# choyingw/SynergyNet

Hardware: AMD Instinct MI355X
Metric: faces/sec (120x120, 68-lmk + 53215-vert) (higher is better)
Workload: dtype f32 (fp16x2 split operands, fp32 accumulate)

## Files before the change

synergynet_amd/csrc/fused_block_lb.hip:

```cpp
#include "syn_internal.h"

#include <cstdio>
#include <cstdlib>

namespace syn {

typedef float f32x4 __attribute__((ext_vector_type(4)));
typedef float f32x2 __attribute__((ext_vector_type(2)));
typedef unsigned u32x4 __attribute__((ext_vector_type(4)));
typedef unsigned u32x2 __attribute__((ext_vector_type(2)));
typedef _Float16 f16x8 __attribute__((ext_vector_type(8)));
typedef _Float16 f16x2 __attribute__((ext_vector_type(2)));

namespace {
__device__ __forceinline__ void split2h(float x0, float x1, unsigned &a, unsigned &b) {
    a = __builtin_bit_cast(unsigned, __builtin_amdgcn_cvt_pkrtz(x0, x1));
    float r0, r1;
    asm("v_fma_mix_f32 %0, %1, -1.0, %2 op_sel_hi:[1,0,0]" : "=v"(r0) : "v"(a), "v"(x0));
    asm("v_fma_mix_f32 %0, %1, -1.0, %2 op_sel:[1,0,0] op_sel_hi:[1,0,0]" : "=v"(r1) : "v"(a), "v"(x1));
    b = __builtin_bit_cast(unsigned, __builtin_amdgcn_cvt_pkrtz(r0, r1));
}
__device__ __forceinline__ void split2v(float x0, float x1, u32x4 (&pc)[2], int d) {
    unsigned a, b;
    split2h(x0, x1, a, b);
    pc[0][d] = a; pc[1][d] = b;
}
__device__ __forceinline__ f32x4 mfmal(u32x4 a, u32x4 b, f32x4 c) {
    return __builtin_amdgcn_mfma_f32_16x16x32_f16(__builtin_bit_cast(f16x8, a), __builtin_bit_cast(f16x8, b), c, 0, 0, 0);
}
__device__ __forceinline__ void mac3x4(const u32x4 (&a0)[2], const u32x4 (&b0)[2], f32x4 &c0, const u32x4 (&a1)[2], const u32x4 (&b1)[2], f32x4 &c1,
                                       const u32x4 (&a2)[2], const u32x4 (&b2)[2], f32x4 &c2, const u32x4 (&a3)[2], const u32x4 (&b3)[2], f32x4 &c3) {
    constexpr int PA[3] = {1, 0, 0}, PB[3] = {0, 1, 0};
#pragma unroll
    for (int j = 0; j < 3; ++j) {
        c0 = mfmal(a0[PA[j]], b0[PB[j]], c0);
        c1 = mfmal(a1[PA[j]], b1[PB[j]], c1);
        c2 = mfmal(a2[PA[j]], b2[PB[j]], c2);
        c3 = mfmal(a3[PA[j]], b3[PB[j]], c3);
    }
}
__device__ __forceinline__ u32x4 bload4(__amdgpu_buffer_rsrc_t rs, unsigned voff, int soff) {
    return __builtin_amdgcn_raw_buffer_load_b128(rs, voff, soff, 0);
}
__device__ __forceinline__ f32x4 bload4f(__amdgpu_buffer_rsrc_t rs, unsigned voff, int soff) {
    return __builtin_bit_cast(f32x4, __builtin_amdgcn_raw_buffer_load_b128(rs, voff, soff, 0));
}
template <int CTRL>
__device__ __forceinline__ float dpp1(float x) {
    return __builtin_bit_cast(float, __builtin_amdgcn_mov_dpp(__builtin_bit_cast(int, x), CTRL, 0xf, 0xf, true));
}
template <int CTRL>
__device__ __forceinline__ f32x2 dpp2(f32x2 v) {
    f32x2 r;
    r[0] = dpp1<CTRL>(v[0]);
    r[1] = dpp1<CTRL>(v[1]);
    return r;
}
__device__ __forceinline__ float relu01(float d, float m) { return __builtin_amdgcn_fmed3f(d * m, 0.0f, 1.0f); }
__device__ __forceinline__ f32x2 pk_fma_clamp01(f32x2 a, f32x2 b, f32x2 c) {
    f32x2 r;
    asm("v_pk_fma_f32 %0, %1, %2, %3 clamp" : "=v"(r) : "v"(a), "v"(b), "v"(c));
    return r;
}
constexpr int kRowShr1 = 0x111, kRowShl1 = 0x101, kRowShr8 = 0x118, kRowShl8 = 0x108;
constexpr int kRowShr4 = 0x114, kRowShr5 = 0x115;
}

template <int CIN_, int HID_, int COUT_, bool RES_, int EPF_, int PPF_, int FPW_ = 2, bool S2_ = false, int NS_ = 2>
struct LbCfg {
    static constexpr int CIN = CIN_, HID = HID_, COUT = COUT_, FPW = FPW_;
    static constexpr int PPF = PPF_;
    static constexpr bool TLATE = false;
    static constexpr int EPF = EPF_;
    static constexpr bool RES = RES_;
    static constexpr bool S2 = S2_;
    static constexpr int NB = S2 ? 1 : 4;
    static constexpr int PIXO = NB * 16;
    static constexpr int KE = CIN / 32;
    static constexpr int NG = HID / 32;
    static constexpr int MT = COUT / 16;
    static constexpr int NS = NS_;
    static constexpr int NW = FPW * NS, NT = NW * 64;
    static constexpr int XF_DW = KE * 4 * 2 * 256;
    static constexpr int NSX = NS == 8 ? 4 : NS;
    static constexpr int KT = (MT + NSX - 1) / NSX;
    static constexpr int RED_DW = (NS == 2 ? 1 : NSX) * MT * NB * 256;
    static constexpr int TB_DW = 12 * 32;
    static constexpr int FACE_DW = XF_DW > RED_DW ? XF_DW : RED_DW;
    static constexpr int LDS_DW = FPW * FACE_DW + NW * TB_DW;
    static_assert(CIN % 32 == 0 && HID % 64 == 0 && COUT % 32 == 0, "k32 steps, two streams, two halves of the output tiles");
    static_assert(NS == 2 || (NS == 8 && FPW == 1 && (HID / 32) >= NS), "eight streams: the one-face-per-workgroup schedule of small batches (the four-stream form of round 4 is retired)");
    static_assert(EPF == 1 || EPF == KE, "expand prefetch depth");
    static_assert(!RES || (CIN == COUT && !S2), "residual only on same-width stride-1 blocks");
    static_assert((FPW == 4 || NS >= 4 ? 1 : 2) * LDS_DW * 4 <= 160 * 1024, "one 8-wave or two 4-wave workgroups per CU");
};

#define SYNL_FENCE() do { asm volatile("" ::: "memory"); __builtin_amdgcn_sched_barrier(0); } while (0)

#define SYNL_LAP(i) do { if (PROF) { tn = __builtin_amdgcn_s_memtime(); pt_[i] += tn - tk; tk = tn; } } while (0)

struct LbStageArgs {
    const float *X;
    const unsigned *Weh;
    const float *Tlb;
    const unsigned *Wlb;
    const float *p_shift;
    float *Y;
    float *part = nullptr;
    int gsl = 0;
};

template <class C, class CN, bool FIRST, bool PROF, int FACE_DW, bool STORE = true, bool PARTIAL = false, int RED_OFF = 0>
__device__ __forceinline__ void lb_stage(unsigned *smem, const LbStageArgs &sa, int B, unsigned long long (&pt_)[5], unsigned long long &tk) {
    unsigned long long tn = 0;
    const float *__restrict__ X = sa.X;
    const unsigned *__restrict__ Weh = sa.Weh, *__restrict__ Wlb = sa.Wlb;
    const float *__restrict__ Tlb = sa.Tlb, *__restrict__ p_shift = sa.p_shift;
    float *__restrict__ Y = sa.Y;
    constexpr int KE = C::KE, MT = C::MT, CIN = C::CIN, COUT = C::COUT, NB = C::NB;
    const int tid = threadIdx.x, lane = tid & 63;
    const int wave = __builtin_amdgcn_readfirstlane(tid >> 6);
    const int fl = wave / C::NS, st = wave % C::NS;
    const int f = blockIdx.x * C::FPW + fl;
    const bool real = f < B;
    const int fc = real ? f : B - 1;
    const int n = lane & 15, g = lane >> 4;
    const unsigned l4 = lane * 4, g4 = g * 4;
    unsigned *Xf = smem + fl * FACE_DW;
    constexpr int BPW = 4 / C::NS;
    auto pix_in = [&](int b, int nn) __attribute__((always_inline)) {
        return C::S2 ? 16 * (nn >> 2) + 8 * (b >> 1) + 2 * (nn & 3) + (b & 1) : 32 * (nn >> 3) + (nn & 7) + 8 * b;
    };

    if constexpr (FIRST && C::NS == 8) {
        constexpr int NIT = (KE * 4 + 7) / 8;
        f32x4 xv[NIT][2];
#pragma unroll
        for (int i = 0; i < NIT; ++i) {
            const int it = st + 8 * i, itc = it < KE * 4 ? it : 0;
            const float *src = X + ((size_t)fc * 64 + pix_in(itc & 3, n)) * CIN + 32 * (itc >> 2) + 8 * g;
            xv[i][0] = *(const f32x4 *)src;
            xv[i][1] = *(const f32x4 *)(src + 4);
        }
#pragma unroll
        for (int i = 0; i < NIT; ++i) {
            const int it = st + 8 * i;
            f32x4 a = xv[i][0], b = xv[i][1];
            if (!real) { a = (f32x4){0.f, 0.f, 0.f, 0.f}; b = a; }
            a *= 16.0f; b *= 16.0f;
            u32x4 pc[2];
            split2v(a[0], a[1], pc, 0);
            split2v(a[2], a[3], pc, 1);
            split2v(b[0], b[1], pc, 2);
            split2v(b[2], b[3], pc, 3);
            if (it < KE * 4) {
#pragma unroll
                for (int p = 0; p < 2; ++p) *(u32x4 *)&Xf[(it * 2 + p) * 256 + lane * 4] = pc[p];
            }
        }
    } else if (FIRST) {
        f32x4 xv[KE][BPW][2];
#pragma unroll
        for (int kc = 0; kc < KE; ++kc)
#pragma unroll
            for (int rr = 0; rr < BPW; ++rr) {
                const float *src = X + ((size_t)fc * 64 + pix_in(BPW * st + rr, n)) * CIN + 32 * kc + 8 * g;
                xv[kc][rr][0] = *(const f32x4 *)src;
                xv[kc][rr][1] = *(const f32x4 *)(src + 4);
            }
#pragma unroll
        for (int kc = 0; kc < KE; ++kc)
#pragma unroll
            for (int rr = 0; rr < BPW; ++rr) {
                f32x4 a = xv[kc][rr][0], b = xv[kc][rr][1];
                if (!real) { a = (f32x4){0.f, 0.f, 0.f, 0.f}; b = a; }
                a *= 16.0f; b *= 16.0f;
                u32x4 pc[2];
                split2v(a[0], a[1], pc, 0);
                split2v(a[2], a[3], pc, 1);
                split2v(b[0], b[1], pc, 2);
                split2v(b[2], b[3], pc, 3);
#pragma unroll
                for (int p = 0; p < 2; ++p) *(u32x4 *)&Xf[((kc * 4 + BPW * st + rr) * 2 + p) * 256 + lane * 4] = pc[p];
            }
    }
    const float mL = (C::S2 ? (n & 3) : (n & 7)) != 0 ? 1.f : 0.f, mR = (C::S2 || (n & 7) != 7) ? 1.f : 0.f;
    f32x4 acc[MT][NB];
#pragma unroll
    for (int mt = 0; mt < MT; ++mt)
#pragma unroll
        for (int r = 0; r < NB; ++r) acc[mt][r] = (f32x4){0.f, 0.f, 0.f, 0.f};

    float *Tb = reinterpret_cast<float *>(smem + C::FPW * FACE_DW + wave * C::TB_DW);
    const __amdgpu_buffer_rsrc_t rs_e = __builtin_amdgcn_make_buffer_rsrc(const_cast<unsigned *>(Weh), 0, 0x7fffffff, 0x00027000);
    const __amdgpu_buffer_rsrc_t rs_p = __builtin_amdgcn_make_buffer_rsrc(const_cast<unsigned *>(Wlb), 0, 0x7fffffff, 0x00027000);
    const __amdgpu_buffer_rsrc_t rs_t = __builtin_amdgcn_make_buffer_rsrc(const_cast<float *>(Tlb), 0, 0x7fffffff, 0x00027000);
    const unsigned l16 = lane * 16;
    f32x4 tv[2];
    auto fetch_t = [&](int G) __attribute__((always_inline)) {
        tv[0] = bload4f(rs_t, l16, G * (C::TB_DW * 4));
        tv[1] = bload4f(rs_t, l16 & 511, G * (C::TB_DW * 4) + 1024);
    };
    auto park_t = [&]() __attribute__((always_inline)) {
        *(f32x4 *)&Tb[l4] = tv[0];
        *(f32x4 *)&Tb[256 + (l4 & 127)] = tv[1];
    };
    const float c6e = Tlb[11 * 32], inv_p = Tlb[11 * 32 + 1];
    u32x4 Ae[C::EPF == 1 ? 2 : KE][2][2];
    auto fetch_e = [&](int G, int kc) __attribute__((always_inline)) {
#pragma unroll
        for (int t = 0; t < 2; ++t)
#pragma unroll
            for (int p = 0; p < 2; ++p)
                Ae[kc % (C::EPF == 1 ? 2 : KE)][t][p] = bload4(rs_e, l16, G * (2 * KE * 2048) + ((t * KE + kc) * 2 + p) * 1024);
    };
    const int gb = PARTIAL ? (int)blockIdx.y * sa.gsl : 0, gend = PARTIAL ? gb + sa.gsl : C::NG;
    fetch_t(gb + st);
#pragma unroll
    for (int kc = 0; kc < C::EPF; ++kc) fetch_e(gb + st, kc);
    park_t();
    __syncthreads();
    SYNL_LAP(0);

    for (int G = gb + st; G < gend; G += C::NS) {
        f32x4 D[2][4];
#pragma unroll
        for (int t = 0; t < 2; ++t) {
            const f32x4 es = *(const f32x4 *)&Tb[10 * 32 + 16 * t + g4];
#pragma unroll
            for (int r = 0; r < 4; ++r) D[t][r] = es;
        }
#pragma unroll
        for (int kc = 0; kc < KE; ++kc) {
            if (kc + C::EPF < KE) fetch_e(G, kc + C::EPF);
            constexpr int SL = C::EPF == 1 ? 2 : KE;
#pragma unroll
            for (int r = 0; r < 4; r += 2) {
                u32x4 Bx[2][2];
#pragma unroll
                for (int rr = 0; rr < 2; ++rr)
#pragma unroll
                    for (int p = 0; p < 2; ++p) Bx[rr][p] = *(const u32x4 *)&Xf[((kc * 4 + r + rr) * 2 + p) * 256 + lane * 4];
                mac3x4(Ae[kc % SL][0], Bx[0], D[0][r], Ae[kc % SL][1], Bx[0], D[1][r], Ae[kc % SL][0], Bx[1], D[0][r + 1], Ae[kc % SL][1], Bx[1], D[1][r + 1]);
                SYNL_FENCE();
            }
        }
        if (C::EPF == KE && G + C::NS < gend) {
#pragma unroll
            for (int kc = 0; kc < C::EPF; ++kc) fetch_e(G + C::NS, kc);
        }
        SYNL_FENCE();
        SYNL_LAP(1);
        constexpr int RING = C::S2 ? 4 : C::PPF + 1;
        u32x4 Ap[RING][2];
        auto fetch_p = [&](int mt) __attribute__((always_inline)) {
#pragma unroll
            for (int p = 0; p < 2; ++p) Ap[mt % RING][p] = bload4(rs_p, l16, G * (MT * 2048) + (mt * 2 + p) * 1024);
        };
        u32x4 Bd[NB][2];
#pragma unroll
        for (int th = 0; th < 4; ++th) {
            const int t = th >> 1, hf = th & 1;
            if (th == 3) fetch_p(0);
            const int c0 = 16 * t + 2 * hf;
            f32x2 w[9];
#pragma unroll
            for (int k = 0; k < 9; ++k) w[k] = *(const f32x2 *)&Tb[k * 32 + c0 + g4];
            const f32x2 dsh = *(const f32x2 *)&Tb[9 * 32 + c0 + g4];
            if (C::S2) {
#pragma unroll
                for (int dy = 0; dy < 3; ++dy) { w[3 * dy] *= mL; w[3 * dy + 2] *= mR; }
            }
            f32x2 E[4], O[NB];
#pragma unroll
            for (int r = 0; r < 4; ++r) {
                E[r][0] = relu01(D[t][r][2 * hf], c6e);
                E[r][1] = relu01(D[t][r][2 * hf + 1], c6e);
            }
#pragma unroll
            for (int r = 0; r < NB; ++r) O[r] = dsh;
            if constexpr (C::S2) {
                O[0] += dpp2<kRowShr5>(E[3]) * w[0];
                O[0] += dpp2<kRowShr4>(E[2]) * w[1];
                O[0] += dpp2<kRowShr4>(E[3]) * w[2];
                asm volatile("" : "+v"(O[0]));
                O[0] += dpp2<kRowShr1>(E[1]) * w[3];
                O[0] += E[0] * w[4];
                O[0] += E[1] * w[5];
                asm volatile("" : "+v"(O[0]));
                O[0] += dpp2<kRowShr1>(E[3]) * w[6];
                O[0] += E[2] * w[7];
                O[0] = pk_fma_clamp01(E[3], w[8], O[0]);
            } else {
                const f32x2 mL2 = {mL, mL}, mR2 = {mR, mR};
                f32x2 rowT = E[3], rowB = E[0];
                asm volatile("" : "+v"(rowT), "+v"(rowB));
                rowT = dpp2<kRowShr8>(rowT);
                rowB = dpp2<kRowShl8>(rowB);
#pragma unroll
                for (int r = 0; r < 4; ++r) {
                    const f32x2 &i0 = r == 0 ? rowT : E[r - 1], &i1 = E[r], &i2 = r == 3 ? rowB : E[r + 1];
                    f32x2 A = i0 * w[0], Cc = i0 * w[2], Bc = O[r] + i0 * w[1];
                    A += i1 * w[3]; Bc += i1 * w[4]; Cc += i1 * w[5];
                    A += i2 * w[6]; Bc += i2 * w[7]; Cc += i2 * w[8];
                    Bc += dpp2<kRowShr1>(A) * mL2;
                    O[r] = pk_fma_clamp01(dpp2<kRowShl1>(Cc), mR2, Bc);
                    asm volatile("" : "+v"(O[r]));
                }
            }
#pragma unroll
            for (int r = 0; r < NB; ++r) {
                split2v(O[r][0], O[r][1], Bd[r], th);
                if (hf) {
#pragma unroll
                    for (int p = 0; p < 2; ++p) asm volatile("" : "+v"(Bd[r][p]));
                }
            }
            SYNL_FENCE();
        }
        SYNL_LAP(2);
        const bool more = G + C::NS < gend;
#pragma unroll
        for (int i = 1; i < C::PPF; ++i)
            if (i < MT) fetch_p(i);
        if (more) {
            if (!C::TLATE) fetch_t(G + C::NS);
            if (C::EPF != KE) {
#pragma unroll
                for (int kc = 0; kc < C::EPF; ++kc) fetch_e(G + C::NS, kc);
            }
        }
        if constexpr (C::S2) {
            static_assert(!C::S2 || (C::PPF == 2 && MT % 2 == 0), "output tiles in pairs, two tiles fetched ahead");
#pragma unroll
            for (int mt = 0; mt < MT; mt += 2) {
                if (mt + 2 < MT) { fetch_p(mt + 2); fetch_p(mt + 3); }
                constexpr int PA[3] = {1, 0, 0}, PB[3] = {0, 1, 0};
#pragma unroll
                for (int j = 0; j < 3; ++j) {
                    acc[mt][0] = mfmal(Ap[mt % RING][PA[j]], Bd[0][PB[j]], acc[mt][0]);
                    acc[mt + 1][0] = mfmal(Ap[(mt + 1) % RING][PA[j]], Bd[0][PB[j]], acc[mt + 1][0]);
                }
                SYNL_FENCE();
            }
        } else {
#pragma unroll
            for (int mt = 0; mt < MT; ++mt) {
                if (mt + C::PPF < MT) fetch_p(mt + C::PPF);
                mac3x4(Ap[mt % RING], Bd[0], acc[mt][0], Ap[mt % RING], Bd[1], acc[mt][1], Ap[mt % RING], Bd[2], acc[mt][2], Ap[mt % RING], Bd[3], acc[mt][3]);
                SYNL_FENCE();
            }
        }
        if (more) {
            if (C::TLATE) fetch_t(G + C::NS);
            park_t();
        }
        SYNL_LAP(3);
    }

    float *Red = reinterpret_cast<float *>(Xf + RED_OFF);
    int le = lane;
    asm volatile("" : "+v"(le));
    const int ne = le & 15, ge = le >> 4, pixe = C::S2 ? ne : 32 * (ne >> 3) + (ne & 7);
    const __amdgpu_buffer_rsrc_t rs_x = __builtin_amdgcn_make_buffer_rsrc(const_cast<float *>(X), 0, 0x7fffffff, 0x00027000);
    constexpr int KT = C::KT, NSW = C::NSX;
    f32x4 rs[KT][NB], psh[KT];
#pragma unroll
    for (int i = 0; i < KT; ++i) {
        const int mtk = NSW * i + (st & (NSW - 1));
        const int nch = 16 * (mtk < MT ? mtk : MT - 1) + 4 * ge;
        psh[i] = *(const f32x4 *)&p_shift[nch];
#pragma unroll
        for (int r = 0; r < NB; ++r)
            if (C::RES && !PARTIAL) rs[i][r] = __builtin_bit_cast(f32x4, __builtin_amdgcn_raw_buffer_load_b128(rs_x, (unsigned)(((fc * 64 + pixe + 8 * r) * COUT + nch) * 4), 0, FIRST ? 0 : 1));
    }
    if (RED_OFF == 0) __syncthreads();
    constexpr bool HANDOFF = !__is_same(CN, void);
    f32x4 vout[KT][NB];
    if constexpr (C::NS == 2) {
#pragma unroll
    for (int mt = 0; mt < MT; ++mt) {
        if ((mt & 1) == st) continue;
#pragma unroll
        for (int r = 0; r < NB; ++r) *(f32x4 *)&Red[(((st * (MT / 2) + (mt >> 1)) * NB + r) * 64 + lane) * 4] = acc[mt][r];
    }
    __syncthreads();
#pragma unroll
    for (int mt = 0; mt < MT; ++mt) {
        if ((mt & 1) != st) continue;
        const int nch = 16 * mt + 4 * ge;
#pragma unroll
        for (int r = 0; r < NB; ++r) {
            const f32x4 o = *(const f32x4 *)&Red[((((1 - st) * (MT / 2) + (mt >> 1)) * NB + r) * 64 + lane) * 4];
            f32x4 v = st == 0 ? acc[mt][r] + o : o + acc[mt][r];
            if constexpr (PARTIAL) {
                if (real) *(f32x4 *)&sa.part[(((size_t)blockIdx.y * B + f) * C::PIXO + pixe + 8 * r) * COUT + nch] = v;
                continue;
            }
            v = v * inv_p + psh[mt >> 1];
            if (C::RES) v += rs[mt >> 1][r];
            if (STORE && real) *(f32x4 *)&Y[((size_t)f * C::PIXO + pixe + 8 * r) * COUT + nch] = v;
            if (HANDOFF) vout[mt >> 1][r] = v;
        }
    }
    } else {
        static_assert(!PARTIAL, "the four-stream schedule reduces inside the workgroup");
        if constexpr (C::NS == 8) {
            if (st >= 4) {
#pragma unroll
                for (int mt = 0; mt < MT; ++mt)
// ... 14 lines not shown
            if (mt % NSW == st || st >= NSW) continue;
#pragma unroll
            for (int r = 0; r < NB; ++r) *(f32x4 *)&Red[(((st * MT + mt) * NB + r) * 64 + lane) * 4] = acc[mt][r];
        }
        __syncthreads();
#pragma unroll
        for (int mt = 0; mt < MT; ++mt) {
            if (mt % NSW != st) continue;
            const int nch = 16 * mt + 4 * ge;
#pragma unroll
            for (int r = 0; r < NB; ++r) {
                f32x4 v = st == 0 ? acc[mt][r] : *(const f32x4 *)&Red[(((0 * MT + mt) * NB + r) * 64 + lane) * 4];
#pragma unroll
                for (int so = 1; so < NSW; ++so) v += so == st ? acc[mt][r] : *(const f32x4 *)&Red[(((so * MT + mt) * NB + r) * 64 + lane) * 4];
                v = v * inv_p + psh[mt / NSW];
                if (C::RES) v += rs[mt / NSW][r];
                if (STORE && real) *(f32x4 *)&Y[((size_t)f * C::PIXO + pixe + 8 * r) * COUT + nch] = v;
                if (HANDOFF) vout[mt / NSW][r] = v;
            }
        }
    }
    if constexpr (HANDOFF) {
        static_assert(CN::CIN == COUT && !C::S2, "the next block of the chain takes this block's output (8x8)");
        if (RED_OFF == 0) __syncthreads();
#pragma unroll
        for (int mt = 0; mt < MT; ++mt) {
            if (mt % NSW != st) continue;
            const int kc = mt >> 1, lg = (2 * (mt & 1) + (ge >> 1)) * 16, dw = 2 * (ge & 1);
#pragma unroll
            for (int r = 0; r < 4; ++r) {
                const f32x4 v = real ? vout[mt / NSW][r] * 16.0f : (f32x4){0.f, 0.f, 0.f, 0.f};
                unsigned a0, b0, a1, b1;
                split2h(v[0], v[1], a0, b0);
                split2h(v[2], v[3], a1, b1);
                const int bn = CN::S2 ? 2 * (r & 1) + (ne & 1) : r;
                const int nn = CN::S2 ? 4 * ((r >> 1) + 2 * (ne >> 3)) + ((ne & 7) >> 1) : ne;
                *(u32x2 *)&Xf[((kc * 4 + bn) * 2 + 0) * 256 + (lg + nn) * 4 + dw] = (u32x2){a0, a1};
                *(u32x2 *)&Xf[((kc * 4 + bn) * 2 + 1) * 256 + (lg + nn) * 4 + dw] = (u32x2){b0, b1};
            }
        }
    }
    SYNL_LAP(4);
}

struct L7 {
    static constexpr int CIN = 32, HID = 192, COUT = 64, NG = 6, MT = 4, H = 15, HO = 8;
    static constexpr int FPW = 2, NW = 4, NT = 256;
    static constexpr int XF_DW = 16 * 2 * 256;
    static constexpr int TB_DW = 12 * 32;
    static constexpr int FACE_DW = XF_DW;
    static constexpr int LDS_DW = FPW * FACE_DW + NW * TB_DW;
};

template <class CN, bool PROF, int FACE_DW>
__device__ __forceinline__ void lb7_stage(unsigned *smem, const LbStageArgs &sa, int B, unsigned long long (&pt_)[5], unsigned long long &tk) {
    unsigned long long tn = 0;
    const float *__restrict__ X = sa.X;
    const float *__restrict__ Tlb = sa.Tlb, *__restrict__ p_shift = sa.p_shift;
    float *__restrict__ Y = sa.Y;
    constexpr int MT = L7::MT, CIN = L7::CIN, COUT = L7::COUT;
    const int tid = threadIdx.x, lane = tid & 63;
    const int wave = __builtin_amdgcn_readfirstlane(tid >> 6);
    const int fl = wave >> 1, st = wave & 1;
    const int f = blockIdx.x * L7::FPW + fl;
    const bool real = f < B;
    const int fc = real ? f : B - 1;
    const int n = lane & 15, g = lane >> 4;
    const unsigned l4 = lane * 4, g4 = g * 4;
    unsigned *Xf = smem + fl * FACE_DW;

#pragma unroll
    for (int hb = 0; hb < 2; ++hb) {
        f32x4 xv[4][2];
        bool ok[4];
#pragma unroll
        for (int b = 0; b < 4; ++b) {
            const int y = 2 * (2 * b + (n >> 3)) + st, x = 2 * (n & 7) + hb;
            ok[b] = real && y < L7::H && x < L7::H;
            const float *src = X + ((size_t)fc * (L7::H * L7::H) + (ok[b] ? y * L7::H + x : 0)) * CIN + 8 * g;
            xv[b][0] = *(const f32x4 *)src;
            xv[b][1] = *(const f32x4 *)(src + 4);
        }
#pragma unroll
        for (int b = 0; b < 4; ++b) {
            f32x4 a = xv[b][0], c = xv[b][1];
            if (!ok[b]) { a = (f32x4){0.f, 0.f, 0.f, 0.f}; c = a; }
            a *= 16.0f; c *= 16.0f;
            u32x4 pc[2];
            split2v(a[0], a[1], pc, 0);
            split2v(a[2], a[3], pc, 1);
            split2v(c[0], c[1], pc, 2);
            split2v(c[2], c[3], pc, 3);
#pragma unroll
            for (int p = 0; p < 2; ++p) *(u32x4 *)&Xf[((((2 * st + hb) * 4 + b) * 2) + p) * 256 + lane * 4] = pc[p];
        }
    }
    const float mL = (n & 7) != 0 ? 1.f : 0.f;
    f32x4 acc[MT][2];
#pragma unroll
    for (int mt = 0; mt < MT; ++mt)
#pragma unroll
        for (int k = 0; k < 2; ++k) acc[mt][k] = (f32x4){0.f, 0.f, 0.f, 0.f};

    float *Tb = reinterpret_cast<float *>(smem + L7::FPW * FACE_DW + wave * L7::TB_DW);
    const __amdgpu_buffer_rsrc_t rs_e = __builtin_amdgcn_make_buffer_rsrc(const_cast<unsigned *>(sa.Weh), 0, 0x7fffffff, 0x00027000);
    const __amdgpu_buffer_rsrc_t rs_p = __builtin_amdgcn_make_buffer_rsrc(const_cast<unsigned *>(sa.Wlb), 0, 0x7fffffff, 0x00027000);
    const __amdgpu_buffer_rsrc_t rs_t = __builtin_amdgcn_make_buffer_rsrc(const_cast<float *>(Tlb), 0, 0x7fffffff, 0x00027000);
    const unsigned l16 = lane * 16;
    f32x4 tv[2];
    auto fetch_t = [&](int G) __attribute__((always_inline)) {
        tv[0] = bload4f(rs_t, l16, G * (L7::TB_DW * 4));
        tv[1] = bload4f(rs_t, l16 & 511, G * (L7::TB_DW * 4) + 1024);
    };
    auto park_t = [&]() __attribute__((always_inline)) {
        *(f32x4 *)&Tb[l4] = tv[0];
        *(f32x4 *)&Tb[256 + (l4 & 127)] = tv[1];
    };
    const float c6e = Tlb[11 * 32], inv_p = Tlb[11 * 32 + 1];
    const float cJ = (n & 7) != 7 ? c6e : 0.f;
    const float cR0 = (st == 1 && n >= 8) ? 0.f : c6e, cR1 = (st == 1 && n >= 8) ? 0.f : cJ;
    u32x4 Ae[2][2];
    auto fetch_e = [&](int G) __attribute__((always_inline)) {
#pragma unroll
        for (int t = 0; t < 2; ++t)
#pragma unroll
            for (int p = 0; p < 2; ++p) Ae[t][p] = bload4(rs_e, l16, G * 4096 + (t * 2 + p) * 1024);
    };
    fetch_t(0);
    fetch_e(0);
    park_t();
    __syncthreads();
    SYNL_LAP(0);

    for (int G = 0; G < L7::NG; ++G) {
        f32x4 D[2][4][3];
#pragma unroll
        for (int t = 0; t < 2; ++t) {
            const f32x4 es = *(const f32x4 *)&Tb[10 * 32 + 16 * t + g4];
#pragma unroll
            for (int c = 0; c < 4; ++c)
#pragma unroll
                for (int k = 0; k < 3; ++k) D[t][c][k] = es;
        }
#pragma unroll
        for (int c = 0; c < 4; ++c) {
            u32x4 Bx[2][2];
#pragma unroll
            for (int k = 0; k < 2; ++k)
#pragma unroll
                for (int p = 0; p < 2; ++p) Bx[k][p] = *(const u32x4 *)&Xf[(((c * 4 + 2 * st + k) * 2) + p) * 256 + lane * 4];
            mac3x4(Ae[0], Bx[0], D[0][c][0], Ae[1], Bx[0], D[1][c][0], Ae[0], Bx[1], D[0][c][1], Ae[1], Bx[1], D[1][c][1]);
            SYNL_FENCE();
        }
        if (st == 1) {
            u32x4 Bx[2][2];
#pragma unroll
            for (int c = 2; c < 4; ++c)
#pragma unroll
                for (int p = 0; p < 2; ++p) Bx[c - 2][p] = *(const u32x4 *)&Xf[(((c * 4 + 1) * 2) + p) * 256 + lane * 4];
            mac3x4(Ae[0], Bx[0], D[0][2][2], Ae[1], Bx[0], D[1][2][2], Ae[0], Bx[1], D[0][3][2], Ae[1], Bx[1], D[1][3][2]);
            SYNL_FENCE();
        }
        SYNL_LAP(1);
        u32x4 Ap[3][2];
        auto fetch_p = [&](int mt) __attribute__((always_inline)) {
#pragma unroll
            for (int p = 0; p < 2; ++p) Ap[mt % 3][p] = bload4(rs_p, l16, G * (MT * 2048) + (mt * 2 + p) * 1024);
        };
        u32x4 Bd[2][2];
#pragma unroll
        for (int th = 0; th < 4; ++th) {
            const int t = th >> 1, hf = th & 1;
            if (th == 3) fetch_p(0);
            const int c0 = 16 * t + 2 * hf;
            f32x2 w[9];
#pragma unroll
            for (int k = 0; k < 9; ++k) w[k] = *(const f32x2 *)&Tb[k * 32 + c0 + g4];
            const f32x2 dsh = *(const f32x2 *)&Tb[9 * 32 + c0 + g4];
#pragma unroll
            for (int dy = 0; dy < 3; ++dy) w[3 * dy] *= mL;
            auto relu = [&](const f32x4 &d, float ceil) __attribute__((always_inline)) {
                f32x2 e;
                e[0] = relu01(d[2 * hf], ceil);
                e[1] = relu01(d[2 * hf + 1], ceil);
                return e;
            };
            f32x2 up2, up3;
            if (st == 1) {
                up2 = dpp2<kRowShl8>(relu(D[t][2][2], c6e));
                up3 = dpp2<kRowShl8>(relu(D[t][3][2], cJ));
            } else {
                up2 = (f32x2){0.f, 0.f}; up3 = up2;
            }
#pragma unroll
            for (int k = 0; k < 2; ++k) {
                const f32x2 E0 = relu(D[t][0][k], c6e), E1 = relu(D[t][1][k], cJ);
                const f32x2 E2 = relu(D[t][2][k], k == 1 ? cR0 : c6e), E3 = relu(D[t][3][k], k == 1 ? cR1 : cJ);
                const f32x2 U2 = dpp2<kRowShr8>(E2) + up2, U3 = dpp2<kRowShr8>(E3) + up3;
                f32x2 O = dsh;
                O += dpp2<kRowShr1>(U3) * w[0];
                O += U2 * w[1];
                O += U3 * w[2];
                asm volatile("" : "+v"(O));
                O += dpp2<kRowShr1>(E1) * w[3];
                O += E0 * w[4];
                O += E1 * w[5];
                asm volatile("" : "+v"(O));
                O += dpp2<kRowShr1>(E3) * w[6];
                O += E2 * w[7];
                O = pk_fma_clamp01(E3, w[8], O);
                split2v(O[0], O[1], Bd[k], th);
                if (k == 0) { up2 = dpp2<kRowShl8>(E2); up3 = dpp2<kRowShl8>(E3); }
            }
            SYNL_FENCE();
        }
        SYNL_LAP(2);
        const bool more = G + 1 < L7::NG;
        fetch_p(1);
        if (more) { fetch_t(G + 1); fetch_e(G + 1); }
#pragma unroll
        for (int mt = 0; mt < MT; ++mt) {
            if (mt + 2 < MT) fetch_p(mt + 2);
            constexpr int PA[3] = {1, 0, 0}, PB[3] = {0, 1, 0};
#pragma unroll
            for (int j = 0; j < 3; ++j) {
                acc[mt][0] = mfmal(Ap[mt % 3][PA[j]], Bd[0][PB[j]], acc[mt][0]);
                acc[mt][1] = mfmal(Ap[mt % 3][PA[j]], Bd[1][PB[j]], acc[mt][1]);
            }
            SYNL_FENCE();
        }
        if (more) park_t();
        SYNL_LAP(3);
    }

    int le = lane;
    asm volatile("" : "+v"(le));
    const int ne = le & 15, ge = le >> 4, ox = ne & 7;
    constexpr bool HANDOFF = !__is_same(CN, void);
    if constexpr (HANDOFF) __syncthreads();
#pragma unroll
    for (int mt = 0; mt < MT; ++mt) {
        const int nch = 16 * mt + 4 * ge;
        const f32x4 psh = *(const f32x4 *)&p_shift[nch];
#pragma unroll
        for (int k = 0; k < 2; ++k) {
            const int oy = 4 * st + 2 * k + (ne >> 3);
            const f32x4 v = acc[mt][k] * inv_p + psh;
            if (real) *(f32x4 *)&Y[((size_t)f * 64 + oy * 8 + ox) * COUT + nch] = v;
            if constexpr (HANDOFF) {
                static_assert(CN::CIN == COUT && !CN::S2, "features.8 takes this block's output");
                const int kc = mt >> 1, lg = (2 * (mt & 1) + (ge >> 1)) * 16, dw = 2 * (ge & 1);
                const int r = 2 * k + (ne >> 3), nn = 8 * st + ox;
                const f32x4 vs = real ? v * 16.0f : (f32x4){0.f, 0.f, 0.f, 0.f};
                unsigned a0, b0, a1, b1;
                split2h(vs[0], vs[1], a0, b0);
                split2h(vs[2], vs[3], a1, b1);
                *(u32x2 *)&Xf[((kc * 4 + r) * 2 + 0) * 256 + (lg + nn) * 4 + dw] = (u32x2){a0, a1};
                *(u32x2 *)&Xf[((kc * 4 + r) * 2 + 1) * 256 + (lg + nn) * 4 + dw] = (u32x2){b0, b1};
            }
        }
    }
    SYNL_LAP(4);
}

template <class CN, int FACE_DW>
__device__ __forceinline__ void lb7_stage8(unsigned *smem, const LbStageArgs &sa, int B) {
    const float *__restrict__ X = sa.X;
    const float *__restrict__ Tlb = sa.Tlb, *__restrict__ p_shift = sa.p_shift;
    float *__restrict__ Y = sa.Y;
    constexpr int MT = L7::MT, CIN = L7::CIN, COUT = L7::COUT;
    const int tid = threadIdx.x, lane = tid & 63;
    const int wave = __builtin_amdgcn_readfirstlane(tid >> 6);
    const int q = wave & 3, hs = wave >> 2;
    const int f = blockIdx.x;
    const bool real = f < B;
    const int fc = real ? f : B - 1;
    const int n = lane & 15, g = lane >> 4;
    const unsigned l4 = lane * 4, g4 = g * 4;
    unsigned *Xf = smem;

    {
        const int c = wave & 3, py = c >> 1, px = c & 1, b0 = 2 * (wave >> 2);
        f32x4 xv[2][2];
        bool ok[2];
#pragma unroll
// ... 134 lines not shown
        if (more) { fetch_t(G + 2); fetch_e(G + 2); }
#pragma unroll
        for (int mt = 0; mt < MT; ++mt) {
            if (mt + 2 < MT) fetch_p(mt + 2);
            constexpr int PA[3] = {1, 0, 0}, PB[3] = {0, 1, 0};
#pragma unroll
            for (int j = 0; j < 3; ++j) acc[mt] = mfmal(Ap[mt % 3][PA[j]], Bd[PB[j]], acc[mt]);
            SYNL_FENCE();
        }
        if (more) park_t();
    }

    float *Ex = reinterpret_cast<float *>(Xf);
    int le = lane;
    asm volatile("" : "+v"(le));
    const int ne = le & 15, ge = le >> 4, ox = ne & 7, oy = 2 * q + (ne >> 3);
    __syncthreads();
    if (hs == 1) {
#pragma unroll
        for (int mt = 0; mt < MT; ++mt) *(f32x4 *)&Ex[((q * MT + mt) * 64 + lane) * 4] = acc[mt];
    }
    __syncthreads();
    f32x4 v[MT];
    if (hs == 0) {
#pragma unroll
        for (int mt = 0; mt < MT; ++mt) {
            const int nch = 16 * mt + 4 * ge;
            v[mt] = (acc[mt] + *(const f32x4 *)&Ex[((q * MT + mt) * 64 + lane) * 4]) * inv_p + *(const f32x4 *)&p_shift[nch];
            if (real) *(f32x4 *)&Y[((size_t)f * 64 + oy * 8 + ox) * COUT + nch] = v[mt];
        }
    }
    static_assert(CN::CIN == COUT && !CN::S2, "features.8 takes this block's output");
    __syncthreads();
    if (hs == 0) {
#pragma unroll
        for (int mt = 0; mt < MT; ++mt) {
            const int kc = mt >> 1, lg = (2 * (mt & 1) + (ge >> 1)) * 16, dw = 2 * (ge & 1);
            const int r = oy & 3, nn = 8 * (oy >> 2) + ox;
            const f32x4 vs = real ? v[mt] * 16.0f : (f32x4){0.f, 0.f, 0.f, 0.f};
            unsigned a0, b0, a1, b1;
            split2h(vs[0], vs[1], a0, b0);
            split2h(vs[2], vs[3], a1, b1);
            *(u32x2 *)&Xf[((kc * 4 + r) * 2 + 0) * 256 + (lg + nn) * 4 + dw] = (u32x2){a0, a1};
            *(u32x2 *)&Xf[((kc * 4 + r) * 2 + 1) * 256 + (lg + nn) * 4 + dw] = (u32x2){b0, b1};
        }
    }
}

template <bool PROF = false>
__global__ __launch_bounds__(L7::NT) __attribute__((amdgpu_waves_per_eu(2, 2)))
void fused_block_lb7_kernel(LbStageArgs sa, int B, unsigned long long *prof = nullptr) {
    unsigned long long pt_[5] = {0, 0, 0, 0, 0}, tk = PROF ? __builtin_amdgcn_s_memtime() : 0ull;
    __shared__ __attribute__((aligned(16))) unsigned smem[L7::LDS_DW];
    lb7_stage<void, PROF, L7::FACE_DW>(smem, sa, B, pt_, tk);
    if (PROF && (threadIdx.x & 63) == 0) {
        for (int i = 0; i < 5; ++i) atomicAdd(&prof[i], pt_[i]);
        atomicAdd(&prof[7], 1ull);
    }
}

template <class C, bool PROF = false, bool PARTIAL = false>
__global__ __launch_bounds__(C::NT) __attribute__((amdgpu_waves_per_eu(2, 2)))
void fused_block_lb_kernel(LbStageArgs sa, int B, unsigned long long *prof = nullptr) {
    unsigned long long pt_[5] = {0, 0, 0, 0, 0}, tk = PROF ? __builtin_amdgcn_s_memtime() : 0ull;
    __shared__ __attribute__((aligned(16))) unsigned smem[C::LDS_DW];
    lb_stage<C, void, true, PROF, C::FACE_DW, true, PARTIAL>(smem, sa, B, pt_, tk);
    if (PROF && (threadIdx.x & 63) == 0) {
        for (int i = 0; i < 5; ++i) atomicAdd(&prof[i], pt_[i]);
        atomicAdd(&prof[7], 1ull);
    }
}

using L8 = LbCfg<      64, 384,  64, true,  2, 3>;
using L11 = LbCfg<     64, 384,  96, false, 2, 3>;
using L12 = LbCfg<     96, 576,  96, true,  1, 3>;
using L14 = LbCfg<     96, 576, 160, false, 1, 2, 2, true>;

struct LbChainArgs { LbStageArgs s[8]; };
constexpr int kChainFaceDw = L7::FACE_DW;
static_assert(L8::FACE_DW <= kChainFaceDw && L11::FACE_DW <= kChainFaceDw && L12::FACE_DW <= kChainFaceDw && L14::FACE_DW <= kChainFaceDw,
              "every stage reuses the fragment buffers of the first");
constexpr int kChainLdsDw = L8::FPW * kChainFaceDw + L8::NW * L8::TB_DW;
static_assert(2 * kChainLdsDw * 4 <= 160 * 1024, "two workgroups per CU");

template <int NG, int KE, int MT>
__device__ __forceinline__ void lb_touch_stage(const LbStageArgs &sa, unsigned gi, unsigned nth, unsigned &sink) {
    l2_touch(sa.Weh, NG * KE * 4096u, gi, nth, sink);
    l2_touch(sa.Wlb, NG * MT * 2048u, gi, nth, sink);
    l2_touch(sa.Tlb, NG * 12u * 32u * 4u, gi, nth, sink);
}
template <bool WITH7, bool WITH14>
__global__ __launch_bounds__(L8::NT) __attribute__((amdgpu_waves_per_eu(2, 2)))
void fused_chain_lb_kernel(LbChainArgs ca, int B) {
    unsigned long long pt_[5] = {0, 0, 0, 0, 0}, tk = 0;
    __shared__ __attribute__((aligned(16))) unsigned smem[kChainLdsDw];
    unsigned sink = 0;
    const unsigned gi = (blockIdx.x >> 3) * (unsigned)L8::NT + threadIdx.x, nth = ((gridDim.x + 7) >> 3) * (unsigned)L8::NT;
    if (WITH7) lb_touch_stage<L7::NG, 1, L7::MT>(ca.s[0], gi, nth, sink);
    lb_touch_stage<L8::NG, L8::KE, L8::MT>(ca.s[1], gi, nth, sink);
    lb_touch_stage<L8::NG, L8::KE, L8::MT>(ca.s[2], gi, nth, sink);
    lb_touch_stage<L8::NG, L8::KE, L8::MT>(ca.s[3], gi, nth, sink);
    lb_touch_stage<L11::NG, L11::KE, L11::MT>(ca.s[4], gi, nth, sink);
    lb_touch_stage<L12::NG, L12::KE, L12::MT>(ca.s[5], gi, nth, sink);
    lb_touch_stage<L12::NG, L12::KE, L12::MT>(ca.s[6], gi, nth, sink);
    if (WITH14) lb_touch_stage<L14::NG, L14::KE, L14::MT>(ca.s[7], gi, nth, sink);
    if constexpr (WITH7) {
        lb7_stage<L8, false, kChainFaceDw>(smem, ca.s[0], B, pt_, tk);
        lb_stage<L8, L8, false, false, kChainFaceDw>(smem, ca.s[1], B, pt_, tk);
    } else
        lb_stage<L8, L8, true, false, kChainFaceDw>(smem, ca.s[1], B, pt_, tk);
    lb_stage<L8, L8, false, false, kChainFaceDw>(smem, ca.s[2], B, pt_, tk);
    lb_stage<L8, L11, false, false, kChainFaceDw>(smem, ca.s[3], B, pt_, tk);
    lb_stage<L11, L12, false, false, kChainFaceDw>(smem, ca.s[4], B, pt_, tk);
    lb_stage<L12, L12, false, false, kChainFaceDw>(smem, ca.s[5], B, pt_, tk);
    if constexpr (WITH14) {
        lb_stage<L12, L14, false, false, kChainFaceDw, false>(smem, ca.s[6], B, pt_, tk);
        lb_stage<L14, void, false, false, kChainFaceDw>(smem, ca.s[7], B, pt_, tk);
    } else
        lb_stage<L12, void, false, false, kChainFaceDw>(smem, ca.s[6], B, pt_, tk);
    l2_touch_done(sink);
}

constexpr int cmax4(int a, int b, int c, int d) { return (a > b ? a : b) > (c > d ? c : d) ? (a > b ? a : b) : (c > d ? c : d); }

using L8e = LbCfg<     64, 384,  64, true,  2, 3, 1, false, 8>;
using L11e = LbCfg<    64, 384,  96, false, 2, 3, 1, false, 8>;
using L12e = LbCfg<    96, 576,  96, true,  1, 3, 1, false, 8>;
using L14e = LbCfg<    96, 576, 160, false, 1, 2, 1, true, 8>;
constexpr int kChainXfDwE = cmax4(L7::XF_DW, L8e::XF_DW, L12e::XF_DW, L14e::XF_DW);
constexpr int kChainRedDwE = cmax4(L8e::RED_DW, L11e::RED_DW, L12e::RED_DW, L14e::RED_DW);
constexpr int kRedOffE = kChainXfDwE;
constexpr int kFaceDwE = kChainXfDwE + kChainRedDwE;
constexpr int kLdsDwE = kFaceDwE + L8e::NW * L8e::TB_DW;
static_assert(kLdsDwE * 4 <= 160 * 1024, "one workgroup per CU");
template <bool WITH7 = false>
__global__ __launch_bounds__(L8e::NT) __attribute__((amdgpu_waves_per_eu(2, 2)))
void fused_chain_lb_small8_kernel(LbChainArgs ca, int B) {
    unsigned long long pt_[5] = {0, 0, 0, 0, 0}, tk = 0;
    __shared__ __attribute__((aligned(16))) unsigned smem[kLdsDwE];
    if constexpr (WITH7) {
        lb7_stage8<L8e, kFaceDwE>(smem, ca.s[0], B);
        lb_stage<L8e, L8e, false, false, kFaceDwE, true, false, kRedOffE>(smem, ca.s[1], B, pt_, tk);
    } else
    lb_stage<L8e, L8e, true, false, kFaceDwE, true, false, kRedOffE>(smem, ca.s[1], B, pt_, tk);
    lb_stage<L8e, L8e, false, false, kFaceDwE, true, false, kRedOffE>(smem, ca.s[2], B, pt_, tk);
    lb_stage<L8e, L11e, false, false, kFaceDwE, true, false, kRedOffE>(smem, ca.s[3], B, pt_, tk);
    lb_stage<L11e, L12e, false, false, kFaceDwE, true, false, kRedOffE>(smem, ca.s[4], B, pt_, tk);
    lb_stage<L12e, L12e, false, false, kFaceDwE, true, false, kRedOffE>(smem, ca.s[5], B, pt_, tk);
    lb_stage<L12e, L14e, false, false, kFaceDwE, false, false, kRedOffE>(smem, ca.s[6], B, pt_, tk);
    lb_stage<L14e, void, false, false, kFaceDwE, true, false, kRedOffE>(smem, ca.s[7], B, pt_, tk);
}

template <class C>
__global__ __launch_bounds__(256) void lb_reduce_kernel(const float *__restrict__ part, int S, const float *__restrict__ Tlb,
                                                        const float *__restrict__ p_shift, const float *__restrict__ X,
                                                        float *__restrict__ Y, int B) {
    constexpr int C4 = C::COUT / 4;
    const long idx = (long)blockIdx.x * 256 + threadIdx.x, total = (long)B * C::PIXO * C4;
    if (idx >= total) return;
    const int c4 = (int)(idx % C4);
    const float inv_p = Tlb[11 * 32 + 1];
    f32x4 a = *(const f32x4 *)&part[(size_t)idx * 4];
    for (int sl = 1; sl < S; ++sl) a += *(const f32x4 *)&part[((size_t)sl * total + idx) * 4];
    f32x4 v = a * inv_p + *(const f32x4 *)&p_shift[4 * c4];
    if (C::RES) v += *(const f32x4 *)&X[(size_t)idx * 4];
    *(f32x4 *)&Y[(size_t)idx * 4] = v;
}

template <class C>
static bool launch_lb_sliced(const FusedBlockArgs &a, int B, hipStream_t s) {
    if (!a.scratch || a.prof) return false;
    const int wg = (B + C::FPW - 1) / C::FPW;
    int S = 0;
    for (int d = 2; d <= C::NG / 2; ++d)
        if (C::NG % d == 0) { S = d; if (wg * d >= 256) break; }
    if (S < 2 || (size_t)S * B * C::PIXO * C::COUT > a.scratch_floats) return false;
    LbStageArgs sa{a.X, a.Alb_e, a.Tlb, a.Alb_p, a.p_shift, a.Y};
    sa.part = a.scratch; sa.gsl = C::NG / S;
    fused_block_lb_kernel<C, false, true><<<dim3(wg, S), C::NT, 0, s>>>(sa, B);
    const long total = (long)B * C::PIXO * (C::COUT / 4);
    lb_reduce_kernel<C><<<(int)((total + 255) / 256), 256, 0, s>>>(a.scratch, S, a.Tlb, a.p_shift, a.X, a.Y, B);
    return true;
}

template <class C>
static void launch_lb(const FusedBlockArgs &a, int B, hipStream_t s) {
    const int grid = (B + C::FPW - 1) / C::FPW;
    const LbStageArgs sa{a.X, a.Alb_e, a.Tlb, a.Alb_p, a.p_shift, a.Y};
    if (a.prof) fused_block_lb_kernel<C, true><<<grid, C::NT, 0, s>>>(sa, B, a.prof);
    else fused_block_lb_kernel<C><<<grid, C::NT, 0, s>>>(sa, B);
}

constexpr int kChainMin = 384;
constexpr int kSmallChainMax = 256;
static bool small_f7() {
    static const bool on = test_knob("small_f7", 1) != 0;
    return on;
}
int lb_chain_mode(int B, bool small) {
    static const int chain = (int)test_knob("lb_chain", 3);
    if (chain <= 0) return 0;
    if (B < kChainMin) return (small && B <= kSmallChainMax) ? (small_f7() ? 3 : 2) : 0;
    return chain > 3 ? 3 : chain;
// ... 57 lines not shown
```

Before: 1.022 million.

## Prefetch next stage's first weights and table during each stage's last group

In the fused chain kernel, each stage's last group is peeled so it can issue buffer loads for the next stage's first expand fragments and table into a shared register struct. The next stage then skips its own cold prologue fetch. This is meant to hide the global-load latency at stage boundaries behind the tail of the previous stage. To make room, the exchange buffer is moved behind the fragment area (RED_OFF offsets) and the chain's face buffer size becomes a max over stages. The cost is more register pressure and an LDS layout that now depends on the offset bounds being correct.

```diff
diff --git a/synergynet_amd/csrc/fused_block_lb.hip b/synergynet_amd/csrc/fused_block_lb.hip
--- a/synergynet_amd/csrc/fused_block_lb.hip
+++ b/synergynet_amd/csrc/fused_block_lb.hip
@@ -2,6 +2,7 @@
 
 #include <cstdio>
 #include <cstdlib>
+#include <type_traits>
 
 namespace syn {
 
@@ -99,6 +100,12 @@
 
 #define SYNL_LAP(i) do { if (PROF) { tn = __builtin_amdgcn_s_memtime(); pt_[i] += tn - tk; tk = tn; } } while (0)
 
+struct LbWarm {
+    f32x4 tv[2];
+    u32x4 Ae[2][2][2];
+};
+struct LbNoNext { static constexpr int TB_DW = 12 * 32, NS = 2, EPF = 1, KE = 1; };
+
 struct LbStageArgs {
     const float *X;
     const unsigned *Weh;
@@ -110,8 +117,12 @@
     int gsl = 0;
 };
 
-template <class C, class CN, bool FIRST, bool PROF, int FACE_DW, bool STORE = true, bool PARTIAL = false, int RED_OFF = 0>
-__device__ __forceinline__ void lb_stage(unsigned *smem, const LbStageArgs &sa, int B, unsigned long long (&pt_)[5], unsigned long long &tk) {
+template <class C, class CN, bool FIRST, bool PROF, int FACE_DW, bool STORE = true, bool PARTIAL = false, int RED_OFF = 0, bool WIN = false, bool WOUT = false>
+__device__ __forceinline__ void lb_stage(unsigned *smem, const LbStageArgs &sa, int B, unsigned long long (&pt_)[5], unsigned long long &tk, LbWarm &wm,
+                                         const LbStageArgs *nx = nullptr) {
+    static_assert(!WOUT || (!__is_same(CN, void) && !PARTIAL && C::NS == 2 && C::NG % C::NS == 0), "the peeled group hands its registers to a next stage of the two-stream chain");
+    static_assert(!WIN || (!FIRST && !PARTIAL), "a warm stage has a predecessor in its launch");
+    using CW = std::conditional_t<__is_same(CN, void), LbNoNext, CN>;
     unsigned long long tn = 0;
     const float *__restrict__ X = sa.X;
     const unsigned *__restrict__ Weh = sa.Weh, *__restrict__ Wlb = sa.Wlb;
@@ -196,7 +207,7 @@
     const __amdgpu_buffer_rsrc_t rs_p = __builtin_amdgcn_make_buffer_rsrc(const_cast<unsigned *>(Wlb), 0, 0x7fffffff, 0x00027000);
     const __amdgpu_buffer_rsrc_t rs_t = __builtin_amdgcn_make_buffer_rsrc(const_cast<float *>(Tlb), 0, 0x7fffffff, 0x00027000);
     const unsigned l16 = lane * 16;
-    f32x4 tv[2];
+    f32x4 (&tv)[2] = wm.tv;
     auto fetch_t = [&](int G) __attribute__((always_inline)) {
         tv[0] = bload4f(rs_t, l16, G * (C::TB_DW * 4));
         tv[1] = bload4f(rs_t, l16 & 511, G * (C::TB_DW * 4) + 1024);
@@ -206,7 +217,8 @@
         *(f32x4 *)&Tb[256 + (l4 & 127)] = tv[1];
     };
     const float c6e = Tlb[11 * 32], inv_p = Tlb[11 * 32 + 1];
-    u32x4 Ae[C::EPF == 1 ? 2 : KE][2][2];
+    static_assert((C::EPF == 1 ? 2 : KE) == 2, "two k32 slots of expand fragments (LbWarm)");
+    u32x4 (&Ae)[2][2][2] = wm.Ae;
     auto fetch_e = [&](int G, int kc) __attribute__((always_inline)) {
 #pragma unroll
         for (int t = 0; t < 2; ++t)
@@ -215,14 +227,30 @@
                 Ae[kc % (C::EPF == 1 ? 2 : KE)][t][p] = bload4(rs_e, l16, G * (2 * KE * 2048) + ((t * KE + kc) * 2 + p) * 1024);
     };
     const int gb = PARTIAL ? (int)blockIdx.y * sa.gsl : 0, gend = PARTIAL ? gb + sa.gsl : C::NG;
-    fetch_t(gb + st);
-#pragma unroll
-    for (int kc = 0; kc < C::EPF; ++kc) fetch_e(gb + st, kc);
+    if (!WIN) {
+        fetch_t(gb + st);
+#pragma unroll
+        for (int kc = 0; kc < C::EPF; ++kc) fetch_e(gb + st, kc);
+    }
     park_t();
     __syncthreads();
     SYNL_LAP(0);
 
-    for (int G = gb + st; G < gend; G += C::NS) {
+    auto group = [&](const int G, auto lastc) __attribute__((always_inline)) {
+        constexpr bool LASTG = decltype(lastc)::value;
+        const bool more = WOUT ? !LASTG : G + C::NS < gend;
+        auto fetch_next_e = [&]() __attribute__((always_inline)) {
+            if constexpr (WOUT) {
+                const __amdgpu_buffer_rsrc_t rs_en = __builtin_amdgcn_make_buffer_rsrc(const_cast<unsigned *>(nx->Weh), 0, 0x7fffffff, 0x00027000);
+#pragma unroll
+                for (int kc = 0; kc < CW::EPF; ++kc)
+#pragma unroll
+                    for (int t = 0; t < 2; ++t)
+#pragma unroll
+                        for (int p = 0; p < 2; ++p)
+                            Ae[kc % 2][t][p] = bload4(rs_en, l16, st * (2 * CW::KE * 2048) + ((t * CW::KE + kc) * 2 + p) * 1024);
+            }
+        };
         f32x4 D[2][4];
 #pragma unroll
         for (int t = 0; t < 2; ++t) {
@@ -245,10 +273,11 @@
                 SYNL_FENCE();
             }
         }
-        if (C::EPF == KE && G + C::NS < gend) {
+        if (C::EPF == KE && more) {
 #pragma unroll
             for (int kc = 0; kc < C::EPF; ++kc) fetch_e(G + C::NS, kc);
         }
+        if constexpr (C::EPF == KE && LASTG) fetch_next_e();
         SYNL_FENCE();
         SYNL_LAP(1);
         constexpr int RING = C::S2 ? 4 : C::PPF + 1;
@@ -319,7 +348,6 @@
             SYNL_FENCE();
         }
         SYNL_LAP(2);
-        const bool more = G + C::NS < gend;
 #pragma unroll
         for (int i = 1; i < C::PPF; ++i)
             if (i < MT) fetch_p(i);
@@ -330,6 +358,13 @@
                 for (int kc = 0; kc < C::EPF; ++kc) fetch_e(G + C::NS, kc);
             }
         }
+        if constexpr (LASTG) {
+            static_assert(CW::TB_DW == C::TB_DW && !C::TLATE, "the next stage's table in this stage's registers");
+            const __amdgpu_buffer_rsrc_t rs_tn = __builtin_amdgcn_make_buffer_rsrc(const_cast<float *>(nx->Tlb), 0, 0x7fffffff, 0x00027000);
+            tv[0] = bload4f(rs_tn, l16, st * (C::TB_DW * 4));
+            tv[1] = bload4f(rs_tn, l16 & 511, st * (C::TB_DW * 4) + 1024);
+            if (C::EPF != KE) fetch_next_e();
+        }
         if constexpr (C::S2) {
             static_assert(!C::S2 || (C::PPF == 2 && MT % 2 == 0), "output tiles in pairs, two tiles fetched ahead");
 #pragma unroll
@@ -356,6 +391,12 @@
             park_t();
         }
         SYNL_LAP(3);
+    };
+    if constexpr (WOUT) {
+        for (int G = st; G < C::NG - C::NS; G += C::NS) group(G, std::false_type{});
+        group(C::NG - C::NS + st, std::true_type{});
+    } else {
+        for (int G = gb + st; G < gend; G += C::NS) group(G, std::false_type{});
     }
 
     float *Red = reinterpret_cast<float *>(Xf + RED_OFF);
@@ -476,8 +517,11 @@
     static constexpr int LDS_DW = FPW * FACE_DW + NW * TB_DW;
 };
 
-template <class CN, bool PROF, int FACE_DW>
-__device__ __forceinline__ void lb7_stage(unsigned *smem, const LbStageArgs &sa, int B, unsigned long long (&pt_)[5], unsigned long long &tk) {
+template <class CN, bool PROF, int FACE_DW, bool WOUT = false>
+__device__ __forceinline__ void lb7_stage(unsigned *smem, const LbStageArgs &sa, int B, unsigned long long (&pt_)[5], unsigned long long &tk, LbWarm &wm,
+                                          const LbStageArgs *nx = nullptr) {
+    static_assert(!WOUT || !__is_same(CN, void), "the peeled group hands its registers to features.8");
+    using CW = std::conditional_t<__is_same(CN, void), LbNoNext, CN>;
     unsigned long long tn = 0;
     const float *__restrict__ X = sa.X;
     const float *__restrict__ Tlb = sa.Tlb, *__restrict__ p_shift = sa.p_shift;
@@ -531,7 +575,7 @@
     const __amdgpu_buffer_rsrc_t rs_p = __builtin_amdgcn_make_buffer_rsrc(const_cast<unsigned *>(sa.Wlb), 0, 0x7fffffff, 0x00027000);
     const __amdgpu_buffer_rsrc_t rs_t = __builtin_amdgcn_make_buffer_rsrc(const_cast<float *>(Tlb), 0, 0x7fffffff, 0x00027000);
     const unsigned l16 = lane * 16;
-    f32x4 tv[2];
+    f32x4 (&tv)[2] = wm.tv;
     auto fetch_t = [&](int G) __attribute__((always_inline)) {
         tv[0] = bload4f(rs_t, l16, G * (L7::TB_DW * 4));
         tv[1] = bload4f(rs_t, l16 & 511, G * (L7::TB_DW * 4) + 1024);
@@ -543,7 +587,7 @@
     const float c6e = Tlb[11 * 32], inv_p = Tlb[11 * 32 + 1];
     const float cJ = (n & 7) != 7 ? c6e : 0.f;
     const float cR0 = (st == 1 && n >= 8) ? 0.f : c6e, cR1 = (st == 1 && n >= 8) ? 0.f : cJ;
-    u32x4 Ae[2][2];
+    u32x4 (&Ae)[2][2] = wm.Ae[0];
     auto fetch_e = [&](int G) __attribute__((always_inline)) {
 #pragma unroll
         for (int t = 0; t < 2; ++t)
@@ -556,7 +600,8 @@
     __syncthreads();
     SYNL_LAP(0);
 
-    for (int G = 0; G < L7::NG; ++G) {
+    auto group = [&](const int G, auto lastc) __attribute__((always_inline)) {
+        constexpr bool LASTG = decltype(lastc)::value;
         f32x4 D[2][4][3];
 #pragma unroll
         for (int t = 0; t < 2; ++t) {
@@ -639,9 +684,23 @@
             SYNL_FENCE();
         }
         SYNL_LAP(2);
-        const bool more = G + 1 < L7::NG;
+        const bool more = WOUT ? !LASTG : G + 1 < L7::NG;
         fetch_p(1);
         if (more) { fetch_t(G + 1); fetch_e(G + 1); }
+        if constexpr (LASTG) {
+            static_assert(CW::TB_DW == L7::TB_DW && CW::NS == 2 && CW::EPF <= 2, "features.8's first group in this stage's registers");
+            const __amdgpu_buffer_rsrc_t rs_tn = __builtin_amdgcn_make_buffer_rsrc(const_cast<float *>(nx->Tlb), 0, 0x7fffffff, 0x00027000);
+            const __amdgpu_buffer_rsrc_t rs_en = __builtin_amdgcn_make_buffer_rsrc(const_cast<unsigned *>(nx->Weh), 0, 0x7fffffff, 0x00027000);
+            tv[0] = bload4f(rs_tn, l16, st * (L7::TB_DW * 4));
+            tv[1] = bload4f(rs_tn, l16 & 511, st * (L7::TB_DW * 4) + 1024);
+#pragma unroll
+            for (int kc = 0; kc < CW::EPF; ++kc)
+#pragma unroll
+                for (int t = 0; t < 2; ++t)
+#pragma unroll
+                    for (int p = 0; p < 2; ++p)
+                        wm.Ae[kc % 2][t][p] = bload4(rs_en, l16, st * (2 * CW::KE * 2048) + ((t * CW::KE + kc) * 2 + p) * 1024);
+        }
 #pragma unroll
         for (int mt = 0; mt < MT; ++mt) {
             if (mt + 2 < MT) fetch_p(mt + 2);
@@ -655,6 +714,12 @@
         }
         if (more) park_t();
         SYNL_LAP(3);
+    };
+    if constexpr (WOUT) {
+        for (int G = 0; G < L7::NG - 1; ++G) group(G, std::false_type{});
+        group(L7::NG - 1, std::true_type{});
+    } else {
+        for (int G = 0; G < L7::NG; ++G) group(G, std::false_type{});
     }
 
     int le = lane;
@@ -895,7 +960,8 @@
 void fused_block_lb7_kernel(LbStageArgs sa, int B, unsigned long long *prof = nullptr) {
     unsigned long long pt_[5] = {0, 0, 0, 0, 0}, tk = PROF ? __builtin_amdgcn_s_memtime() : 0ull;
     __shared__ __attribute__((aligned(16))) unsigned smem[L7::LDS_DW];
-    lb7_stage<void, PROF, L7::FACE_DW>(smem, sa, B, pt_, tk);
+    LbWarm wm;
+    lb7_stage<void, PROF, L7::FACE_DW>(smem, sa, B, pt_, tk, wm);
     if (PROF && (threadIdx.x & 63) == 0) {
         for (int i = 0; i < 5; ++i) atomicAdd(&prof[i], pt_[i]);
         atomicAdd(&prof[7], 1ull);
@@ -907,7 +973,8 @@
 void fused_block_lb_kernel(LbStageArgs sa, int B, unsigned long long *prof = nullptr) {
     unsigned long long pt_[5] = {0, 0, 0, 0, 0}, tk = PROF ? __builtin_amdgcn_s_memtime() : 0ull;
     __shared__ __attribute__((aligned(16))) unsigned smem[C::LDS_DW];
-    lb_stage<C, void, true, PROF, C::FACE_DW, true, PARTIAL>(smem, sa, B, pt_, tk);
+    LbWarm wm;
+    lb_stage<C, void, true, PROF, C::FACE_DW, true, PARTIAL>(smem, sa, B, pt_, tk, wm);
     if (PROF && (threadIdx.x & 63) == 0) {
         for (int i = 0; i < 5; ++i) atomicAdd(&prof[i], pt_[i]);
         atomicAdd(&prof[7], 1ull);
@@ -920,7 +987,12 @@
 using L14 = LbCfg<     96, 576, 160, false, 1, 2, 2, true>;
 
 struct LbChainArgs { LbStageArgs s[8]; };
-constexpr int kChainFaceDw = L7::FACE_DW;
+constexpr int cmax2(int a, int b) { return a > b ? a : b; }
+constexpr int kChainFaceDw = cmax2(L7::FACE_DW, L14::XF_DW + L14::RED_DW);
+constexpr int kRedOff8 = L8::XF_DW, kRedOff14 = L14::XF_DW;
+static_assert(kRedOff8 >= L8::XF_DW && kRedOff8 + L8::RED_DW <= kChainFaceDw, "features.8-10: exchange buffer behind the fragments, inside the face buffer");
+static_assert(L8::XF_DW <= kRedOff8 && L11::XF_DW <= kRedOff8, "features.8-10: the fragments handed to the next stage (features.8 | 11) stay below the exchange buffer");
+static_assert(kRedOff14 >= L14::XF_DW && kRedOff14 + L14::RED_DW <= kChainFaceDw, "features.14: exchange buffer behind the fragments, inside the face buffer (no next stage)");
 static_assert(L8::FACE_DW <= kChainFaceDw && L11::FACE_DW <= kChainFaceDw && L12::FACE_DW <= kChainFaceDw && L14::FACE_DW <= kChainFaceDw,
               "every stage reuses the fragment buffers of the first");
 constexpr int kChainLdsDw = L8::FPW * kChainFaceDw + L8::NW * L8::TB_DW;
@@ -947,20 +1019,22 @@
     lb_touch_stage<L12::NG, L12::KE, L12::MT>(ca.s[5], gi, nth, sink);
     lb_touch_stage<L12::NG, L12::KE, L12::MT>(ca.s[6], gi, nth, sink);
     if (WITH14) lb_touch_stage<L14::NG, L14::KE, L14::MT>(ca.s[7], gi, nth, sink);
+    LbWarm wm;
+    constexpr bool W = true;
     if constexpr (WITH7) {
-        lb7_stage<L8, false, kChainFaceDw>(smem, ca.s[0], B, pt_, tk);
-        lb_stage<L8, L8, false, false, kChainFaceDw>(smem, ca.s[1], B, pt_, tk);
+        lb7_stage<L8, false, kChainFaceDw, W>(smem, ca.s[0], B, pt_, tk, wm, &ca.s[1]);
+        lb_stage<L8, L8, false, false, kChainFaceDw, true, false, kRedOff8, W, W>(smem, ca.s[1], B, pt_, tk, wm, &ca.s[2]);
     } else
-        lb_stage<L8, L8, true, false, kChainFaceDw>(smem, ca.s[1], B, pt_, tk);
-    lb_stage<L8, L8, false, false, kChainFaceDw>(smem, ca.s[2], B, pt_, tk);
-    lb_stage<L8, L11, false, false, kChainFaceDw>(smem, ca.s[3], B, pt_, tk);
-    lb_stage<L11, L12, false, false, kChainFaceDw>(smem, ca.s[4], B, pt_, tk);
-    lb_stage<L12, L12, false, false, kChainFaceDw>(smem, ca.s[5], B, pt_, tk);
+        lb_stage<L8, L8, true, false, kChainFaceDw, true, false, kRedOff8, false, W>(smem, ca.s[1], B, pt_, tk, wm, &ca.s[2]);
+    lb_stage<L8, L8, false, false, kChainFaceDw, true, false, kRedOff8, W, W>(smem, ca.s[2], B, pt_, tk, wm, &ca.s[3]);
+    lb_stage<L8, L11, false, false, kChainFaceDw, true, false, kRedOff8, W, W>(smem, ca.s[3], B, pt_, tk, wm, &ca.s[4]);
+    lb_stage<L11, L12, false, false, kChainFaceDw, true, false, 0, W, W>(smem, ca.s[4], B, pt_, tk, wm, &ca.s[5]);
+    lb_stage<L12, L12, false, false, kChainFaceDw, true, false, 0, W, W>(smem, ca.s[5], B, pt_, tk, wm, &ca.s[6]);
     if constexpr (WITH14) {
-        lb_stage<L12, L14, false, false, kChainFaceDw, false>(smem, ca.s[6], B, pt_, tk);
-        lb_stage<L14, void, false, false, kChainFaceDw>(smem, ca.s[7], B, pt_, tk);
+        lb_stage<L12, L14, false, false, kChainFaceDw, false, false, 0, W, W>(smem, ca.s[6], B, pt_, tk, wm, &ca.s[7]);
+        lb_stage<L14, void, false, false, kChainFaceDw, true, false, kRedOff14, W>(smem, ca.s[7], B, pt_, tk, wm);
     } else
-        lb_stage<L12, void, false, false, kChainFaceDw>(smem, ca.s[6], B, pt_, tk);
+        lb_stage<L12, void, false, false, kChainFaceDw, true, false, 0, W>(smem, ca.s[6], B, pt_, tk, wm);
     l2_touch_done(sink);
 }
 
@@ -981,17 +1055,18 @@
 void fused_chain_lb_small8_kernel(LbChainArgs ca, int B) {
     unsigned long long pt_[5] = {0, 0, 0, 0, 0}, tk = 0;
     __shared__ __attribute__((aligned(16))) unsigned smem[kLdsDwE];
+    LbWarm wm;
     if constexpr (WITH7) {
         lb7_stage8<L8e, kFaceDwE>(smem, ca.s[0], B);
-        lb_stage<L8e, L8e, false, false, kFaceDwE, true, false, kRedOffE>(smem, ca.s[1], B, pt_, tk);
+        lb_stage<L8e, L8e, false, false, kFaceDwE, true, false, kRedOffE>(smem, ca.s[1], B, pt_, tk, wm);
     } else
-    lb_stage<L8e, L8e, true, false, kFaceDwE, true, false, kRedOffE>(smem, ca.s[1], B, pt_, tk);
-    lb_stage<L8e, L8e, false, false, kFaceDwE, true, false, kRedOffE>(smem, ca.s[2], B, pt_, tk);
-    lb_stage<L8e, L11e, false, false, kFaceDwE, true, false, kRedOffE>(smem, ca.s[3], B, pt_, tk);
-    lb_stage<L11e, L12e, false, false, kFaceDwE, true, false, kRedOffE>(smem, ca.s[4], B, pt_, tk);
-    lb_stage<L12e, L12e, false, false, kFaceDwE, true, false, kRedOffE>(smem, ca.s[5], B, pt_, tk);
-    lb_stage<L12e, L14e, false, false, kFaceDwE, false, false, kRedOffE>(smem, ca.s[6], B, pt_, tk);
-    lb_stage<L14e, void, false, false, kFaceDwE, true, false, kRedOffE>(smem, ca.s[7], B, pt_, tk);
+    lb_stage<L8e, L8e, true, false, kFaceDwE, true, false, kRedOffE>(smem, ca.s[1], B, pt_, tk, wm);
+    lb_stage<L8e, L8e, false, false, kFaceDwE, true, false, kRedOffE>(smem, ca.s[2], B, pt_, tk, wm);
+    lb_stage<L8e, L11e, false, false, kFaceDwE, true, false, kRedOffE>(smem, ca.s[3], B, pt_, tk, wm);
+    lb_stage<L11e, L12e, false, false, kFaceDwE, true, false, kRedOffE>(smem, ca.s[4], B, pt_, tk, wm);
+    lb_stage<L12e, L12e, false, false, kFaceDwE, true, false, kRedOffE>(smem, ca.s[5], B, pt_, tk, wm);
+    lb_stage<L12e, L14e, false, false, kFaceDwE, false, false, kRedOffE>(smem, ca.s[6], B, pt_, tk, wm);
+    lb_stage<L14e, void, false, false, kFaceDwE, true, false, kRedOffE>(smem, ca.s[7], B, pt_, tk, wm);
 }
 
 template <class C>
```

After: 1.022 million (median of 2 runs). No clear change (+0.0%).
